# tenpy/cyten

Measured on AMD Instinct MI355X. Metric: block-sparse tdot+SVD GFLOP/s (fp64), higher is better.
Workload: dtype f64

## Files before the change

cyten_amd/csrc/blocked_qr.h:

```cpp
#pragma once
#include "common.h"

namespace cyb {

constexpr int NBK = 32;

struct BqrMat {
    double* Ac;
    int64_t ld;
    int32_t m, n, k;
    double* V;
    double* T;
    double* tau;
    double* scratch;
    int64_t scr_half;
    int64_t scr_total = 0;
    int32_t v_zeroed = 0;
    double* ctl = nullptr;
    double* parts = nullptr;
    double stop_rel2 = 0.0;
    int32_t reflect_always = 0;
};

size_t bqr_aux_bytes(int64_t m, int64_t n, int64_t ld, int64_t kc);
size_t bqr_carve(BqrMat& q, char* base, int64_t kc);

int bqr_strip_slots(int64_t rows);

int bqr_factor(cyb_ctx_t ctx, const std::vector<BqrMat>& mats);

struct BqrTarget {
    int32_t mat;
    double* C;
    int64_t ldc;
    int32_t kc;
    int32_t n_pan = -1;
};
int bqr_apply_q(cyb_ctx_t ctx, const std::vector<BqrMat>& mats, const std::vector<BqrTarget>& targets);
int bqr_apply_q_pair(cyb_ctx_t ctx, const std::vector<BqrMat>& mats, const std::vector<BqrTarget>& targets, size_t n_first);

struct XposeDesc {
    const double* in;
    double* out;
    int64_t ldi, ldo;
    int32_t R, C, upper, rlim;
    int32_t plain, pad;
    const int32_t* idx = nullptr;
};
int xpose_batched(cyb_ctx_t ctx, const std::vector<XposeDesc>& descs);
struct EyeDesc {
    double* C;
    int64_t ld;
    int32_t m, kc;
    int32_t col0, pad;
};
int eye_cols_batched(cyb_ctx_t ctx, const std::vector<EyeDesc>& descs);

}
```

cyten_amd/csrc/blocked_qr.hip:

```cpp
#include "blocked_qr.h"

#include <algorithm>
#include <cstdlib>
#include <utility>

namespace cyb {
namespace {

#define GLOBAL_AS __attribute__((address_space(1)))
typedef GLOBAL_AS double* gp;
typedef const GLOBAL_AS double* gcp;
typedef double d4 __attribute__((ext_vector_type(4)));

constexpr int PNT = 512;
constexpr int PNW = PNT / 64;

__device__ __forceinline__ double wave_sum(double v)
{
#pragma unroll
    for (int o = 32; o > 0; o >>= 1) v += __shfl_xor(v, o);
    return v;
}

struct PanelDesc {
    double* Ac;
    double* V;
    double* T;
    double* tau;
    int64_t ld;
    int32_t m, j0, pw, pad;
    double* ctl = nullptr;
    const double* parts = nullptr;
    double rel2 = 0.0;
    int32_t n_parts = 0, step = 0;
};
constexpr int PANEL_V_ZEROED = 1;
constexpr int PANEL_REFLECT_ALWAYS = 2;

__global__ void __launch_bounds__(PNT) qr_panel_kernel(const PanelDesc* __restrict__ descs)
{
    __shared__ double red[PNW];
    __shared__ double s_tau, s_scale;
    __shared__ double Ts[NBK][NBK + 1];
    __shared__ double z[NBK];
    __shared__ double taus[NBK];
    const PanelDesc d = descs[blockIdx.x];
    const int tid = threadIdx.x, lane = tid & 63, wave = tid >> 6;
    gp Ac = (gp)d.Ac;
    gp V = (gp)d.V;
    const int64_t ld = d.ld;
    const int m = d.m, j0 = d.j0, pw = d.pw;
    for (int e = tid; e < NBK * (NBK + 1); e += PNT) (&Ts[0][0])[e] = 0.0;

    for (int jj = 0; jj < pw; ++jj) {
        const int col = j0 + jj;
        gp x = Ac + (int64_t)col * ld + col;
        const int L = m - col;
        double mx = 0.0;
        for (int i = 1 + tid; i < L; i += PNT) mx = fmax(mx, fabs(x[i]));
#pragma unroll
        for (int o = 32; o > 0; o >>= 1) mx = fmax(mx, __shfl_xor(mx, o));
        if (lane == 0) red[wave] = mx;
        __syncthreads();
        mx = 0.0;
#pragma unroll
        for (int q = 0; q < PNW; ++q) mx = fmax(mx, red[q]);
        __syncthreads();
        double ss = 0.0;
        if (mx > 1e-290) {
            const double inv = 1.0 / mx;
            for (int i = 1 + tid; i < L; i += PNT) {
                const double t = x[i] * inv;
                ss += t * t;
            }
        }
        ss = wave_sum(ss);
        if (lane == 0) red[wave] = ss;
        __syncthreads();
        if (tid == 0) {
            double tot = 0.0;
            for (int q = 0; q < PNW; ++q) tot += red[q];
            const double xnorm = mx * sqrt(tot);
            const double alpha = x[0];
            double t = 0.0, scale = 0.0, beta = alpha;
            if (xnorm != 0.0) {
                beta = -copysign(hypot(alpha, xnorm), alpha);
// ... 291 lines not shown
        gcp src = (gcp)Ac + (int64_t)j0 * ld + (ok ? row : j0);
#pragma unroll
        for (int c = 0; c < NBK; ++c) P[q][c] = src[(int64_t)(c < pw ? c : pw - 1) * ld];
#pragma unroll
        for (int c = 0; c < NBK; ++c) {
            asm volatile("" : "+v"(P[q][c]));
            P[q][c] = (ok && c < pw) ? P[q][c] : 0.0;
        }
    }
    for (int e = tid; e < NBK * (NBK + 1); e += NT) (&sh.Zs[0][0])[e] = 0.0;
    __syncthreads();

    panel_steps<RPT, NT>(P, sh, d, tid, std::make_integer_sequence<int, NBK>{});
#pragma unroll
    for (int q = 0; q < RPT; ++q) {
        const int row = j0 + tid + NT * q;
        if (row < m) {
            gp pa = Ac + (int64_t)j0 * ld + row;
            gp pv = V + (int64_t)j0 * ld + row;
#pragma unroll
            for (int c = 0; c < NBK; ++c)
                if (c < pw) {
                    pa[(int64_t)c * ld] = P[q][c];
                    pv[(int64_t)c * ld] = (q > 0 || tid > c) ? P[q][c] : (tid == c ? 1.0 : 0.0);
                }
        }
    }
    for (int64_t e = tid; e < ((d.pad & PANEL_V_ZEROED) ? 0 : (int64_t)j0 * pw); e += NT) {
        const int c = (int)(e / j0), row = (int)(e % j0);
        V[(int64_t)(j0 + c) * ld + row] = 0.0;
    }
    __syncthreads();
    if (tid < NBK) {
        double trow[NBK];
#pragma unroll
        for (int j = 0; j < NBK; ++j) {
            double acc = 0.0;
#pragma unroll
            for (int l = 0; l < j; ++l) acc += trow[l] * sh.Zs[l][j];
            const double tj = j < pw ? sh.taus[j] : 0.0;
            trow[j] = (tid < j) ? -tj * acc : (tid == j ? tj : 0.0);
            sh.Ts[tid][j] = trow[j];
        }
    }
    __syncthreads();

    for (int e = tid; e < NBK * NBK; e += NT) ((gp)d.T)[e] = sh.Ts[e / NBK][e % NBK];
}

template <int NT, typename Desc>
__device__ __forceinline__ bool panel_stop_check(const Desc& d, double* red, int tid, bool writer = true)
{
    if (!d.ctl) return false;
    gp ctl = (gp)d.ctl;
    const double stopped = ctl[0];
    if (stopped != 0.0) return (double)d.step >= stopped - 1.0;
    if (d.n_parts <= 0) return false;
    gcp parts = (gcp)d.parts;
    double t = 0.0;
    for (int i = tid; i < d.n_parts; i += NT) t += parts[i];
#pragma unroll
    for (int o = 32; o > 0; o >>= 1) t += __shfl_xor(t, o);
    if ((tid & 63) == 0) red[tid >> 6] = t;
    __syncthreads();
    double sum = 0.0;
#pragma unroll
    for (int w = 0; w < NT / 64; ++w) sum += red[w];
    const double ref = fmax(ctl[1], sum);
    const bool stop = sum <= d.rel2 * ref;
    __syncthreads();
    if (tid == 0 && writer) {
        if (stop) ctl[0] = (double)d.step + 1.0;
        else ctl[1] = ref;
    }
    return stop;
}

__global__ void __launch_bounds__(RP_NT) qr_panel_reg_kernel(const PanelDesc* __restrict__ descs)
{
    __shared__ PanelShared sh;
    const PanelDesc d = descs[blockIdx.x];
    if (panel_stop_check<RP_NT>(d, &sh.wsum[0][0], (int)threadIdx.x)) return;
    panel_reg_body<RP_RPT>(d, sh, (int)threadIdx.x);
}
struct PanelDescM {
    double* Ac;
    double* V;
    double* T;
    double* tau;
    double* xchg;
    unsigned int* ticket;
    unsigned int* err;
    int64_t ld;
    int32_t m, j0, pw, vzero;
    int32_t wg, n_wg, pad0, pad1;
    double* ctl = nullptr;
    const double* parts = nullptr;
    double rel2 = 0.0;
    int32_t n_parts = 0, step = 0;
};
constexpr int RPM_ROWS = RP_NT * RP_RPT;

template <int JJ>
__device__ __forceinline__ void panel_step_multi(double (&P)[RP_RPT][NBK], PanelShared& sh, const PanelDescM& d, int tid)
{
    if (JJ >= d.pw) return;
    const int lane = tid & 63, wave = tid >> 6;
    const int j0 = d.j0, rbase = d.j0 + d.wg * RPM_ROWS;
    const int prow = j0 + JJ;
    constexpr int pb = JJ & 1;
#pragma unroll
    for (int h = 0; h < 2; ++h) {
        double part[16];
#pragma unroll
        for (int c = 0; c < 16; ++c) part[c] = 0.0;
#pragma unroll
        for (int q = 0; q < RP_RPT; ++q) {
            const int row = rbase + tid + RP_NT * q;
            const double x = (row <= prow) ? 0.0 : P[q][JJ];
#pragma unroll
            for (int c = 0; c < 16; ++c) part[c] += x * P[q][h * 16 + c];
        }
        const double r = reduce_scatter16(part, lane);
        if ((lane & 3) == 0) {
            const int idx = ((lane >> 5) & 1) * 8 + ((lane >> 4) & 1) * 4 + ((lane >> 3) & 1) * 2 + ((lane >> 2) & 1);
            sh.wred[pb][wave][h * 16 + idx] = r;
        }
    }
#pragma unroll
    for (int q = 0; q < RP_RPT; ++q)
        if (rbase + tid + RP_NT * q == prow) {
#pragma unroll
            for (int c = 0; c < NBK; ++c) sh.rowb[pb][c] = P[q][c];
        }
    __syncthreads();
    if (tid < NBK) {
        double t = 0.0;
#pragma unroll
        for (int w = 0; w < RP_NW; ++w) t += sh.wred[pb][w][tid];
        double* slot = d.xchg + ((size_t)JJ * d.n_wg + d.wg) * 64;
        __hip_atomic_store(slot + tid, t, __ATOMIC_RELAXED, __HIP_MEMORY_SCOPE_AGENT);
        if (d.wg == 0) __hip_atomic_store(slot + 32 + tid, sh.rowb[pb][tid], __ATOMIC_RELAXED, __HIP_MEMORY_SCOPE_AGENT);
        asm volatile("s_waitcnt vmcnt(0)" ::: "memory");
        if (tid == 0) {
            __hip_atomic_fetch_add(d.ticket + JJ, 1u, __ATOMIC_RELAXED, __HIP_MEMORY_SCOPE_AGENT);
            const unsigned long long t0 = wall_clock64();
            while (__hip_atomic_load(d.ticket + JJ, __ATOMIC_RELAXED, __HIP_MEMORY_SCOPE_AGENT) < (unsigned int)d.n_wg) {
                if (wall_clock64() - t0 > 100000000ull || __hip_atomic_load(d.err, __ATOMIC_RELAXED, __HIP_MEMORY_SCOPE_AGENT)) {
                    __hip_atomic_store(d.err, 1u, __ATOMIC_RELAXED, __HIP_MEMORY_SCOPE_AGENT);
                    break;
                }
            }
        }
        asm volatile("" ::: "memory");
        __builtin_amdgcn_wave_barrier();
        double tot = 0.0;
        for (int w = 0; w < d.n_wg; ++w)
            tot += __hip_atomic_load(d.xchg + ((size_t)JJ * d.n_wg + w) * 64 + tid, __ATOMIC_RELAXED, __HIP_MEMORY_SCOPE_AGENT);
        sh.wsum[pb][tid] = tot;
        sh.rowb[pb][tid] = __hip_atomic_load(d.xchg + (size_t)JJ * d.n_wg * 64 + 32 + tid, __ATOMIC_RELAXED, __HIP_MEMORY_SCOPE_AGENT);
    }
    __syncthreads();
    const double alpha = sh.rowb[pb][JJ];
    const double xn2 = fma(alpha * alpha, (d.vzero & PANEL_REFLECT_ALWAYS) ? 1e-40 : 0.0, sh.wsum[pb][JJ]);
    double tau = 0.0, scale = 0.0, beta = alpha;
    if (xn2 > 1e-290) {
// ... 687 lines not shown
#pragma unroll
        for (int q = 0; q < 4; ++q) {
            const int c = c0 + ty + 8 * q, r = r0 + tx;
            tile[ty + 8 * q][tx] = (c < d.C && r < d.R) ? in[(int64_t)(d.idx ? cidx[ty + 8 * q] : c) * d.ldi + r] : 0.0;
        }
        __syncthreads();
#pragma unroll
        for (int q = 0; q < 4; ++q) {
            const int r = r0 + ty + 8 * q, c = c0 + tx;
            if (r < d.R && c < d.C) {
                double v = tile[tx][ty + 8 * q];
                if (d.upper && (r > c || r >= d.rlim)) v = 0.0;
                out[(int64_t)r * d.ldo + c] = v;
            }
        }
    }
}

__global__ void __launch_bounds__(256) eye_cols_kernel(const EyeDesc* __restrict__ descs)
{
    const EyeDesc d = descs[blockIdx.y];
    gp C = (gp)d.C;
    const int64_t tot = (int64_t)d.m * d.kc;
    for (int64_t e = (int64_t)blockIdx.x * 256 + threadIdx.x; e < tot; e += (int64_t)gridDim.x * 256) {
        const int64_t c = e / d.m, i = e % d.m;
        C[c * d.ld + i] = (i == c + d.col0) ? 1.0 : 0.0;
    }
}

}

int xpose_batched(cyb_ctx_t ctx, const std::vector<XposeDesc>& descs)
{
    if (descs.empty()) return CYB_OK;
    void* d = nullptr;
    CYB_TRY(ctx->upload(descs.data(), sizeof(XposeDesc) * descs.size(), &d));
    hipLaunchKernelGGL(xpose_kernel, dim3(helper_grid_x(descs.size()), (unsigned)descs.size()), dim3(256), 0, ctx->stream, static_cast<const XposeDesc*>(d));
    CYB_HIP(hipGetLastError());
    return CYB_OK;
}

int eye_cols_batched(cyb_ctx_t ctx, const std::vector<EyeDesc>& descs)
{
    if (descs.empty()) return CYB_OK;
    void* d = nullptr;
    CYB_TRY(ctx->upload(descs.data(), sizeof(EyeDesc) * descs.size(), &d));
    hipLaunchKernelGGL(eye_cols_kernel, dim3(64, (unsigned)descs.size()), dim3(256), 0, ctx->stream, static_cast<const EyeDesc*>(d));
    CYB_HIP(hipGetLastError());
    return CYB_OK;
}

constexpr int kWSplit = 8;
static inline int w_split(int64_t mr)
{
    static const int env = getenv("CYB_QR_WSPLIT") ? atoi(getenv("CYB_QR_WSPLIT")) : 0;
    if (env > 0) return (int)std::min<int64_t>(std::min(env, kWSplit), std::max<int64_t>(1, (mr + 255) / 256));
    return mr >= 2600 ? 4 : mr >= 1800 ? 3 : mr >= 700 ? 2 : 1;
}

static inline bool use_strips()
{
    static const bool off = getenv("CYB_QR_GEMM_UPDATE") != nullptr;
    return !off;
}
static void add_strips(std::vector<StripDesc>& out, double* C, int64_t ldc, int64_t ncols, const double* V, int64_t ldv,
                       const double* T, int64_t mr, int pw, int transT, int64_t next_tag = -1)
{
    for (int64_t c0 = 0; c0 < ncols; c0 += NBK)
        out.push_back(StripDesc{C + (size_t)c0 * ldc, V, T, ldc, ldv, (int32_t)mr, (int32_t)std::min<int64_t>(NBK, ncols - c0), pw, transT,
                                c0 == 0 && next_tag >= 0 ? next_tag + 1 : 0});
}
static void sort_strips(std::vector<StripDesc>& v)
{
    std::stable_sort(v.begin(), v.end(), [](const StripDesc& a, const StripDesc& b) { return a.mr > b.mr; });
}

constexpr int kChunkRowsMin = 192;
static const int kChunkRowsChoices[] = {192, 256, 384, 512, 768, 1024, 1536};
static int strip_split_mode()
{
    static const int v = getenv("CYB_QR_CHUNK_ROWS") ? atoi(getenv("CYB_QR_CHUNK_ROWS")) : -1;
    return v < 0 ? -1 : v / 16 * 16;
}
int bqr_strip_slots(int64_t rows)
{
    if (strip_split_mode() == 0) return 1;
    const int ch = strip_split_mode() > 0 ? std::min(strip_split_mode(), kChunkRowsMin) : kChunkRowsMin;
    return (int)std::max<int64_t>(1, (rows + ch - 1) / ch);
}
static int strip_chunk_share(int mr, int ch)
{
    if (ch <= 0 || mr <= ch) return std::max(mr, 1);
    const int ns = (mr + ch - 1) / ch;
    return ((mr + ns - 1) / ns + 15) / 16 * 16;
}
static int strip_chunks(int mr, int ch)
{
    const int share = strip_chunk_share(mr, ch);
    return std::max(1, (mr + share - 1) / share);
}
static int choose_chunk_rows(const std::vector<std::pair<int, int>>& strips, int n_cu)
{
    const int mode = strip_split_mode();
    if (mode == 0) return 0;
    if (mode > 0) return mode;
    int64_t n_strips = 0;
    for (const auto& s : strips) n_strips += s.second;
    if (n_strips == 0 || n_strips * 4 > (int64_t)n_cu * 3) return 0;
    static const int ch_min = getenv("CYB_QR_CHUNK_MIN") ? atoi(getenv("CYB_QR_CHUNK_MIN")) : kChunkRowsMin;
    for (int ch : kChunkRowsChoices) {
        if (ch < ch_min) continue;
        int64_t tot = 0;
        bool any = false;
        for (const auto& s : strips) {
            const int c = strip_chunks(s.first, ch);
            tot += (int64_t)c * s.second;
            any = any || c > 1;
        }
        if (tot <= n_cu) return any ? ch : 0;
    }
    return 0;
}
static void make_chunks(const std::vector<StripDesc>& sd, double* wbase, int ch, std::vector<ChunkDesc>& out)
{
    out.clear();
    size_t slot_base = 0;
    for (const StripDesc& d : sd) {
        const int share = strip_chunk_share(d.mr, ch), nch = strip_chunks(d.mr, ch);
        for (int sl = 0; sl < nch; ++sl) {
            const int r0 = sl * share;
            out.push_back(ChunkDesc{d.C + r0, d.V + r0, d.T, wbase + slot_base * (size_t)(NBK * NBK), d.ldc, d.ldv, std::min(share, d.mr - r0), d.nc, d.pw,
                                    d.transT, sl, nch, r0, d.step, d.ctl, d.part_out ? d.part_out + sl : nullptr});
        }
        slot_base += (size_t)nch;
    }
}

static int wide_mode()
{
    static const int v = getenv("CYB_QR_APPLY_WIDE") ? (atoi(getenv("CYB_QR_APPLY_WIDE")) != 0 ? 1 : 0) : -1;
    return v;
}
static int wide_width()
{
    static const int v = [] {
        const int e = getenv("CYB_QR_APPLY_WIDTH") ? atoi(getenv("CYB_QR_APPLY_WIDTH")) : 128;
        return (e == 64 || e == 256) ? e : 128;
    }();
    return v;
}
constexpr int64_t kWideMinK = 256, kWideMinKc = 256, kWideMinCols = 4096;
static bool wide_target(const BqrMat& q, const BqrTarget& t)
{
    const int mode = wide_mode();
    if (mode == 0 || q.k <= NBK || t.kc <= 0) return false;
    if (q.ctl && q.stop_rel2 > 0.0 && t.n_pan < 0) return false;
    if (mode == 1) return true;
    return q.k >= kWideMinK && t.kc >= kWideMinKc;
}
static size_t scratch_doubles(int64_t m, int64_t n, int64_t kc)
{
    const size_t strips = (size_t)(1 + kWSplit) * NBK * (size_t)std::max<int64_t>(std::max(n, kc), 1);
    const size_t wide = (size_t)w_split(m) * (size_t)wide_width() * (size_t)std::max<int64_t>(kc, 1);
    return std::max(strips, wide);
}

// ... 33 lines not shown
    const bool strips = use_strips();
    const bool lookahead = !strips && want_la && max_pan >= 6 && ctx->aux(&side) == CYB_OK;
    struct Step {
        size_t off_pd = 0, off_pdr = 0;
        unsigned n_pd = 0, n_pdr = 0;
        GemmStaged s1, s3;
        GemmStaged r1, r3;
        bool has_rest = false;
        size_t off_sd = 0;
        unsigned n_sd = 0;
        bool fused = false;
        bool norm = false;
        unsigned n_la = 0;
        size_t off_pn = 0;
        size_t off_cd = 0;
        unsigned n_cd = 0;
        int wave = 0;
        size_t off_pdm = 0;
        unsigned n_pdm = 0;
    };
    std::vector<Step> steps;
    std::vector<char> image;
    auto put = [&image](const void* src, size_t bytes) {
        const size_t off = (image.size() + 255) / 256 * 256;
        image.resize(off + bytes);
        memcpy(image.data() + off, src, bytes);
        return off;
    };
    static const bool no_fuse = getenv("CYB_QR_FUSE") == nullptr;
    static const int fuse_rows = getenv("CYB_QR_FUSE_ROWS") ? atoi(getenv("CYB_QR_FUSE_ROWS")) : 768;
    std::vector<char> fused(mats.size(), 0);
    static const bool la_on = getenv("CYB_QR_LA") && atoi(getenv("CYB_QR_LA")) != 0;
    static const int la_min_rows = getenv("CYB_QR_LA_MIN") ? atoi(getenv("CYB_QR_LA_MIN")) : 4 * RP_WAVE_ROWS;
    unsigned int* la_flags = nullptr;
    const int la_err = (int)mats.size();
    bool la_used = false;
    static const bool no_multi = getenv("CYB_QR_NOMULTI") != nullptr;
    std::vector<size_t> x_off(mats.size(), 0);
    size_t x_bytes = 0, n_multi_wg = 0;
    const size_t t_bytes = (sizeof(unsigned int) * NBK * mats.size() + 255) / 256 * 256;
    for (size_t qi = 0; qi < mats.size(); ++qi) {
        const int wmax = (mats[qi].m + RPM_ROWS - 1) / RPM_ROWS;
        if (mats[qi].m > RPM_ROWS && std::min(mats[qi].m, mats[qi].n) > 0) {
            x_off[qi] = t_bytes + 256 + x_bytes;
            x_bytes += sizeof(double) * NBK * (size_t)wmax * 64;
            n_multi_wg += (size_t)wmax;
        }
    }
    const bool multi = !no_multi && x_bytes > 0 && n_multi_wg <= (size_t)ctx->n_cu;
    char* xbase = nullptr;
    bool la_any = false;
    if (la_on && use_strips())
        for (const auto& q : mats) la_any = la_any || (q.k > NBK && q.m - NBK > la_min_rows);
    if (multi || la_any) {
        const size_t x_total = multi ? (t_bytes + 256 + x_bytes + 255) / 256 * 256 : 0;
        void* xw = nullptr;
        CYB_TRY(ctx->workspace(x_total + 256 + sizeof(unsigned int) * (mats.size() + 1), &xw, 3));
        xbase = static_cast<char*>(xw);
        if (multi) CYB_HIP(hipMemsetAsync(xbase + t_bytes, 0, 256, ctx->stream));
        if (la_any) {
            la_flags = reinterpret_cast<unsigned int*>(xbase + x_total);
            CYB_HIP(hipMemsetAsync(la_flags, 0, sizeof(unsigned int) * (mats.size() + 1), ctx->stream));
        }
    }
    const bool multi_ok = multi;
    static const bool no_stop = getenv("CYB_QR_NOSTOP") != nullptr;
    static const bool no_reg_g = getenv("CYB_QR_PANEL_GLOBAL") != nullptr;
    auto stoppable = [&](const BqrMat& q) {
        return !no_stop && strips && !no_reg_g && q.ctl && q.parts && q.stop_rel2 > 0.0 && (q.m <= RP_NT * RP_RPT || multi_ok);
    };
    const bool split = strips && strip_split_mode() != 0 && no_fuse && !la_on;
    double* wsplit = nullptr;
    if (split) {
        size_t n_ch = 0;
        for (const auto& q : mats) n_ch += (size_t)((q.n + NBK - 1) / NBK) * (size_t)bqr_strip_slots(q.m);
        void* w = nullptr;
        CYB_TRY(ctx->workspace(sizeof(double) * NBK * NBK * std::max<size_t>(n_ch, 1), &w, 4));
        wsplit = static_cast<double*>(w);
    }
    std::vector<int> n_parts_prev(mats.size(), 0);
    static const int stop_every = std::max(1, getenv("CYB_QR_STOP_EVERY") ? atoi(getenv("CYB_QR_STOP_EVERY")) : 2);
    bool all_done = false;
    int last_rest = -1;
    const int side_cu = ctx->n_cu - (ctx->n_cu + 15) / 16;
    int chunk = lookahead ? max_pan : 2;
    for (int c0 = 0; c0 < max_pan && !all_done; c0 += chunk, chunk *= 3) {
    const int c1 = std::min(max_pan, c0 + chunk);
    steps.clear();
    image.clear();
    for (int p = c0; p < c1; ++p) {
        std::vector<PanelDesc> pd, pd_reg, pd_next;
        std::vector<PanelDescM> pdm;
        std::vector<StripDesc> sd;
        GemmBatch g1, g3, h1, h3;
        int n_active = 0;
        int max_m = 0;
        for (const auto& q : mats)
            if (p * NBK < q.k) max_m = std::max(max_m, q.m);
        const bool step_fuse = !no_fuse && max_m <= fuse_rows;
        const bool step_la = la_on && strips && !step_fuse && la_flags != nullptr;
        bool step_has_la = false;
        bool step_norm = false;
        int step_ch = 0;
        if (split && !step_fuse) {
            std::vector<std::pair<int, int>> cnt;
            for (const auto& q : mats) {
                const int j0 = p * NBK;
                if (j0 >= q.k) continue;
                const int64_t nt = q.n - (j0 + std::min(NBK, q.k - j0));
                if (nt > 0) cnt.push_back({q.m - j0, (int)((nt + NBK - 1) / NBK)});
            }
            step_ch = choose_chunk_rows(cnt, ctx->n_cu);
        }
        for (size_t qi = 0; qi < mats.size(); ++qi) {
            const auto& q = mats[qi];
            const int j0 = p * NBK;
            if (j0 >= q.k) continue;
            ++n_active;
            const int pw = std::min(NBK, q.k - j0);
            static const bool no_reg = getenv("CYB_QR_PANEL_GLOBAL") != nullptr;
            if (fused[qi]) fused[qi] = 0;
            else if (!no_reg && q.m - j0 <= RP_NT * RP_RPT) {
                pd_reg.push_back(PanelDesc{q.Ac, q.V, q.T + (size_t)p * NBK * NBK, q.tau, q.ld, q.m, j0, pw, pflags(q)});
                if (stoppable(q)) {
                    PanelDesc& d = pd_reg.back();
                    d.ctl = q.ctl;
                    d.parts = q.parts;
                    d.rel2 = q.stop_rel2;
                    d.n_parts = n_parts_prev[qi];
                    d.step = p;
                }
            } else if (multi && !no_reg) {
                const int n_wg = (q.m - j0 + RPM_ROWS - 1) / RPM_ROWS;
                for (int w = 0; w < n_wg; ++w)
                {
                    pdm.push_back(PanelDescM{q.Ac, q.V, q.T + (size_t)p * NBK * NBK, q.tau, reinterpret_cast<double*>(xbase + x_off[qi]),
                                             reinterpret_cast<unsigned int*>(xbase) + qi * NBK, reinterpret_cast<unsigned int*>(xbase + t_bytes),
                                             q.ld, q.m, j0, pw, pflags(q), w, n_wg, 0, 0});
                    if (stoppable(q)) {
                        PanelDescM& d = pdm.back();
                        d.ctl = q.ctl;
                        d.parts = q.parts;
                        d.rel2 = q.stop_rel2;
                        d.n_parts = n_parts_prev[qi];
                        d.step = p;
                    }
                }
            } else
                pd.push_back(PanelDesc{q.Ac, q.V, q.T + (size_t)p * NBK * NBK, q.tau, q.ld, q.m, j0, pw, pflags(q) & PANEL_REFLECT_ALWAYS});
            const int j1 = j0 + pw;
            const int64_t nt = q.n - j1, mr = q.m - j0;
            const int parts_lag = n_parts_prev[qi];
            n_parts_prev[qi] = 0;
            if (nt <= 0) continue;
            double* W1 = q.scratch + q.scr_half;
            const double* Vp = q.V + (size_t)j0 * q.ld + j0;
            const double* Tp = q.T + (size_t)p * NBK * NBK;
            if (strips) {
                int64_t tag = -1;
                if (step_fuse && !no_reg && !stoppable(q) && j1 < q.k && q.m - j1 <= RP_NT * RP_RPT_FUSED) {
                    tag = (int64_t)pd_next.size();
                    pd_next.push_back(PanelDesc{q.Ac, q.V, q.T + (size_t)(p + 1) * NBK * NBK, q.tau, q.ld, q.m, j1, std::min(NBK, q.k - j1), pflags(q)});
                    fused[qi] = 1;
                } else if (step_la && !no_reg && j1 < q.k && q.m - j1 <= RP_NT * RP_RPT && q.m - j1 > la_min_rows) {
                    tag = (int64_t)pd_next.size();
                    pd_next.push_back(PanelDesc{q.Ac, q.V, q.T + (size_t)(p + 1) * NBK * NBK, q.tau, q.ld, q.m, j1, std::min(NBK, q.k - j1), pflags(q)});
                    if (stoppable(q)) {
                        const bool measure = p % stop_every == stop_every - 1;
                        PanelDesc& d = pd_next.back();
                        d.ctl = q.ctl;
                        d.parts = q.parts;
                        d.rel2 = q.stop_rel2;
                        d.n_parts = measure ? 0 : parts_lag;
                        d.step = p + 1;
                    }
                    fused[qi] = 1;
                    step_has_la = true;
                }
                const size_t s_begin = sd.size();
                add_strips(sd, q.Ac + (size_t)j1 * q.ld + j0, q.ld, nt, Vp, q.ld, Tp, mr, pw, 1, tag);
                if (stoppable(q)) {
                    const bool measure = p % stop_every == stop_every - 1;
                    const int nch = strip_chunks((int)mr, step_ch);
                    for (size_t si = s_begin; si < sd.size(); ++si) {
                        sd[si].ctl = q.ctl;
                        sd[si].part_out = measure ? q.parts + (si - s_begin) * (size_t)nch : nullptr;
                        sd[si].step = p;
                    }
                    if (measure) {
                        n_parts_prev[qi] = (int)(sd.size() - s_begin) * nch;
                        step_norm = true;
                    }
                }
                continue;
            }
            const int ns = w_split(mr);
            const int64_t chunk = ((mr + ns - 1) / ns + 15) / 16 * 16;
            const int64_t nn = lookahead ? std::min<int64_t>(NBK, nt) : nt;
            auto add = [&](GemmBatch& a1, GemmBatch& a3, int64_t c0, int64_t nc, size_t scr_off) {
                if (nc <= 0) return;
                double* At = q.Ac + (size_t)(j1 + c0) * q.ld + j0;
                const int32_t seg0 = (int32_t)a3.segs.size();
                for (int sidx = 0; sidx < ns; ++sidx) {
                    const int64_t r0 = chunk * sidx, rows = std::min(chunk, mr - r0);
                    if (rows <= 0) break;
                    double* W2s = W1 + (size_t)sidx * q.scr_half + scr_off;
                    a1.add_post(W2s, pw, nc, nc, Vp + r0, q.ld, 1, At + r0, 1, q.ld, rows, 1.0, 0.0, Tp, 1, NBK);
                    a3.segs.push_back(cyb_gemm_seg{W2s, Vp, pw, 1, nc, q.ld, 1});
                }
                a3.probs.push_back(cyb_gemm_prob{At, nc, mr, q.ld, seg0, (int32_t)a3.segs.size(), -1.0, 1.0});
            };
            add(g1, g3, 0, nn, 0);
            add(h1, h3, nn, nt - nn, (size_t)NBK * NBK);
        }
        if (n_active == 0) {
            all_done = true;
            break;
        }
        Step st;
        st.n_pd = (unsigned)pd.size();
        st.n_pdr = (unsigned)pd_reg.size();
        if (st.n_pd) st.off_pd = put(pd.data(), sizeof(PanelDesc) * pd.size());
        if (st.n_pdr) st.off_pdr = put(pd_reg.data(), sizeof(PanelDesc) * pd_reg.size());
        st.n_pdm = (unsigned)pdm.size();
        if (st.n_pdm) st.off_pdm = put(pdm.data(), sizeof(PanelDescM) * pdm.size());
        static const bool no_wave = getenv("CYB_QR_NOWAVE") != nullptr;
        int max_rows = 0;
        for (const auto& d : pd_reg) max_rows = std::max(max_rows, d.m - d.j0);
        st.wave = (no_wave || st.n_pdr == 0) ? 0 : max_rows <= RP_WAVE_ROWS ? 1 : max_rows <= 2 * RP_WAVE_ROWS ? 2 : max_rows <= 4 * RP_WAVE_ROWS ? 4 : 0;
        if (!sd.empty()) {
            sort_strips(sd);
            st.n_sd = (unsigned)sd.size();
            st.fused = !pd_next.empty() && !step_has_la;
            st.norm = step_norm;
            const size_t off_pn = pd_next.empty() ? 0 : put(pd_next.data(), sizeof(PanelDesc) * pd_next.size());
            const size_t off_sd = (image.size() + 255) / 256 * 256;
            if (step_has_la) {
                st.n_la = (unsigned)pd_next.size();
                st.off_pn = off_pn;
                la_used = true;
            } else
                for (auto& d : sd)
                    if (d.next_off) d.next_off = (int64_t)(off_pn + (size_t)(d.next_off - 1) * sizeof(PanelDesc)) - (int64_t)off_sd;
            st.off_sd = put(sd.data(), sizeof(StripDesc) * sd.size());
            if (step_ch > 0 && !st.fused && !st.n_la) {
                std::vector<ChunkDesc> cd;
                make_chunks(sd, wsplit, step_ch, cd);
                st.n_cd = (unsigned)cd.size();
                st.off_cd = put(cd.data(), sizeof(ChunkDesc) * cd.size());
            }
        }
        if (!g1.empty()) {
            CYB_TRY(g1.stage(ctx, image, st.s1));
            CYB_TRY(g3.stage(ctx, image, st.s3));
        }
        if (!h1.empty()) {
            CYB_TRY(h1.stage(ctx, image, st.r1));
            CYB_TRY(h3.stage(ctx, image, st.r3));
            st.has_rest = true;
        }
        steps.push_back(st);
    }
    if (steps.empty()) break;
    void* d_image = nullptr;
    CYB_TRY(ctx->upload(image.data(), image.size(), &d_image));
    char* dbase = static_cast<char*>(d_image);
    if (lookahead) CYB_TRY(ctx->events(2 * steps.size()));
    for (size_t p = 0; p < steps.size(); ++p) {
        const Step& st = steps[p];
        if (st.n_pd)
            hipLaunchKernelGGL(qr_panel_kernel, dim3(st.n_pd), dim3(PNT), 0, ctx->stream,
                               reinterpret_cast<const PanelDesc*>(dbase + st.off_pd));
        if (st.n_pdm) {
            CYB_HIP(hipMemsetAsync(xbase, 0, t_bytes, ctx->stream));
            hipLaunchKernelGGL(qr_panel_multi_kernel, dim3(st.n_pdm), dim3(RP_NT), 0, ctx->stream,
                               reinterpret_cast<const PanelDescM*>(dbase + st.off_pdm));
        }
        if (st.n_pdr && st.wave == 1)
            hipLaunchKernelGGL(qr_panel_wave_kernel, dim3(st.n_pdr), dim3(64), 0, ctx->stream,
                               reinterpret_cast<const PanelDesc*>(dbase + st.off_pdr));
        else if (st.n_pdr && st.wave == 2)
            hipLaunchKernelGGL(qr_panel_wave2_kernel, dim3(st.n_pdr), dim3(128), 0, ctx->stream,
                               reinterpret_cast<const PanelDesc*>(dbase + st.off_pdr));
        else if (st.n_pdr && st.wave == 4)
            hipLaunchKernelGGL(qr_panel_wave4_kernel, dim3(st.n_pdr), dim3(256), 0, ctx->stream,
                               reinterpret_cast<const PanelDesc*>(dbase + st.off_pdr));
        else if (st.n_pdr)
            hipLaunchKernelGGL(qr_panel_reg_kernel, dim3(st.n_pdr), dim3(RP_NT), 0, ctx->stream,
                               reinterpret_cast<const PanelDesc*>(dbase + st.off_pdr));
        CYB_HIP(hipGetLastError());
        if (lookahead && st.has_rest) {
            hipEvent_t evP = ctx->ev_pool[2 * p], evR = ctx->ev_pool[2 * p + 1];
            CYB_HIP(hipEventRecord(evP, ctx->stream));
            CYB_HIP(hipStreamWaitEvent(side, evP, 0));
            CYB_TRY(gemm_launch_staged(ctx, st.r1, d_image, side, side_cu));
            CYB_TRY(gemm_launch_staged(ctx, st.r3, d_image, side, side_cu));
            CYB_HIP(hipEventRecord(evR, side));
            if (last_rest >= 0) CYB_HIP(hipStreamWaitEvent(ctx->stream, ctx->ev_pool[2 * (size_t)last_rest + 1], 0));
            last_rest = (int)p;
        } else if (lookahead && last_rest >= 0) {
            CYB_HIP(hipStreamWaitEvent(ctx->stream, ctx->ev_pool[2 * (size_t)last_rest + 1], 0));
            last_rest = -1;
        }
        if (st.n_sd) {
            const StripDesc* sdp = reinterpret_cast<const StripDesc*>(dbase + st.off_sd);
            const PanelDesc* pnp = reinterpret_cast<const PanelDesc*>(dbase + st.off_pn);
            const unsigned la_tag = (unsigned)(c0 + (int)p + 1);
            const PanelDesc* no_pn = nullptr;
            unsigned int* no_fl = nullptr;
            if (st.n_cd) {
                const ChunkDesc* cdp = reinterpret_cast<const ChunkDesc*>(dbase + st.off_cd);
                hipLaunchKernelGGL(strip_w1_kernel, dim3(st.n_cd), dim3(ST_NT), 0, ctx->stream, cdp);
                if (st.norm) hipLaunchKernelGGL(strip_apply_kernel<true>, dim3(st.n_cd), dim3(ST_NT), 0, ctx->stream, cdp);
                else hipLaunchKernelGGL(strip_apply_kernel<false>, dim3(st.n_cd), dim3(ST_NT), 0, ctx->stream, cdp);
            } else if (st.n_la && st.norm)
                hipLaunchKernelGGL((reflector_strip_kernel<false, true, true>), dim3(st.n_sd + st.n_la), dim3(ST_NT), 0, ctx->stream, sdp,
                                   (int)st.n_sd, pnp, la_flags, la_tag, la_err);
            else if (st.n_la)
                hipLaunchKernelGGL((reflector_strip_kernel<false, false, true>), dim3(st.n_sd + st.n_la), dim3(ST_NT), 0, ctx->stream, sdp,
                                   (int)st.n_sd, pnp, la_flags, la_tag, la_err);
            else if (st.fused)
                hipLaunchKernelGGL(reflector_strip_kernel<true>, dim3(st.n_sd), dim3(ST_NT), 0, ctx->stream, sdp, (int)st.n_sd, no_pn, no_fl, 0u, 0);
            else if (st.norm)
                hipLaunchKernelGGL((reflector_strip_kernel<false, true>), dim3(st.n_sd), dim3(ST_NT), 0, ctx->stream, sdp, (int)st.n_sd, no_pn, no_fl, 0u, 0);
            else
                hipLaunchKernelGGL(reflector_strip_kernel<false>, dim3(st.n_sd), dim3(ST_NT), 0, ctx->stream, sdp, (int)st.n_sd, no_pn, no_fl, 0u, 0);
            CYB_HIP(hipGetLastError());
        }
        CYB_TRY(gemm_launch_staged(ctx, st.s1, d_image));
        CYB_TRY(gemm_launch_staged(ctx, st.s3, d_image));
    }
    }
    if (last_rest >= 0) CYB_HIP(hipStreamWaitEvent(ctx->stream, ctx->ev_pool[2 * (size_t)last_rest + 1], 0));
    if (la_used) {
        unsigned int h_err = 0;
        CYB_HIP(hipMemcpyAsync(&h_err, la_flags + la_err, sizeof(unsigned int), hipMemcpyDeviceToHost, ctx->stream));
        CYB_HIP(hipStreamSynchronize(ctx->stream));
        if (h_err) {
            set_error("blocked QR: a look-ahead panel workgroup waited more than a second for its strip");
            return CYB_ERR_HIP;
        }
    }
    if (multi) {
        unsigned int h_err = 0;
        CYB_HIP(hipMemcpyAsync(&h_err, xbase + t_bytes, sizeof(unsigned int), hipMemcpyDeviceToHost, ctx->stream));
        CYB_HIP(hipStreamSynchronize(ctx->stream));
        if (h_err) {
            set_error("blocked QR: a workgroup of the multi-workgroup panel kernel waited more than a second for its partners");
            return CYB_ERR_HIP;
        }
    }
    return CYB_OK;
}

static int apply_q_strips(cyb_ctx_t ctx, const std::vector<BqrMat>& mats, const std::vector<BqrTarget>& targets)
{
    int max_pan = 0;
    for (const auto& t : targets) max_pan = std::max(max_pan, (mats[(size_t)t.mat].k + NBK - 1) / NBK);
    const bool strips = use_strips();
    struct Step {
        GemmStaged s1, s3;
        size_t off_sd = 0;
        unsigned n_sd = 0;
        size_t off_cd = 0;
        unsigned n_cd = 0;
    };
    const bool split = strips && strip_split_mode() != 0;
    double* wsplit = nullptr;
    if (split) {
        size_t n_ch = 0;
        for (const auto& t : targets) n_ch += (size_t)((t.kc + NBK - 1) / NBK) * (size_t)bqr_strip_slots(mats[(size_t)t.mat].m);
        void* w = nullptr;
        CYB_TRY(ctx->workspace(sizeof(double) * NBK * NBK * std::max<size_t>(n_ch, 1), &w, 4));
        wsplit = static_cast<double*>(w);
    }
    std::vector<Step> steps;
    std::vector<char> image;
    int chunk = 2;
    for (int c0 = max_pan - 1; c0 >= 0; c0 -= chunk, chunk *= 3) {
    const int c1 = std::max(-1, c0 - chunk);
    steps.clear();
    image.clear();
    for (int p = c0; p > c1; --p) {
        GemmBatch g1, g3;
        std::vector<StripDesc> sd;
        for (const auto& t : targets) {
            const BqrMat& q = mats[(size_t)t.mat];
            const int j0 = p * NBK;
            if (j0 >= q.k || t.kc <= 0) continue;
            const int pw = std::min(NBK, q.k - j0);
            const int64_t mr = q.m - j0;
            double* W1 = q.scratch + q.scr_half;
            CYB_REQUIRE((int64_t)NBK * t.kc <= q.scr_half, "bqr_apply_q: target wider than the carved scratch");
            const double* Vp = q.V + (size_t)j0 * q.ld + j0;
            double* Ct = t.C + j0;
            const double* Tp = q.T + (size_t)p * NBK * NBK;
            if (strips) {
                const size_t s_begin = sd.size();
                add_strips(sd, Ct, t.ldc, t.kc, Vp, q.ld, Tp, mr, pw, 0);
                if (q.ctl && q.stop_rel2 > 0.0)
                    for (size_t si = s_begin; si < sd.size(); ++si) {
                        sd[si].ctl = q.ctl;
                        sd[si].step = p;
                    }
                continue;
            }
            const int ns = w_split(mr);
            const int64_t chunk = ((mr + ns - 1) / ns + 15) / 16 * 16;
            const int32_t seg0 = (int32_t)g3.segs.size();
            for (int sidx = 0; sidx < ns; ++sidx) {
                const int64_t r0 = chunk * sidx, rows = std::min(chunk, mr - r0);
                if (rows <= 0) break;
                double* W2s = W1 + (size_t)sidx * q.scr_half;
                g1.add_post(W2s, pw, t.kc, t.kc, Vp + r0, q.ld, 1, Ct + r0, 1, t.ldc, rows, 1.0, 0.0, Tp, NBK, 1);
                g3.segs.push_back(cyb_gemm_seg{W2s, Vp, pw, 1, t.kc, q.ld, 1});
// ... 252 lines not shown
```

cyten_amd/csrc/qr_householder.hip:

```cpp
#include "blocked_qr.h"

#include <algorithm>
#include <cstdlib>

namespace {

#define GLOBAL_AS __attribute__((address_space(1)))
typedef GLOBAL_AS double* gp;
typedef const GLOBAL_AS double* gcp;

constexpr int QNT = 512;
constexpr int QNW = QNT / 64;

struct QrWork {
    const double* A;
    int64_t lda;
    int32_t m, n, k, kq;
    double* Ac;
    double* Qc;
    double* tau;
    double* Q;
    int64_t ldq;
    double* R;
    int64_t ldr;
// ... 110 lines not shown
    for (int64_t e = tid; e < (int64_t)m * kq; e += QNT) {
        const int i = (int)(e / kq), c = (int)(e % kq);
        ((gp)w.Q)[(int64_t)i * w.ldq + c] = Qc[(int64_t)c * m + i];
    }
}

}

static constexpr int64_t kBlockedMin = 96;

static int qr_blocked(cyb_ctx_t ctx, const std::vector<cyb_qr_desc>& ds)
{
    using namespace cyb;
    if (ds.empty()) return CYB_OK;
    auto al = [](size_t b) { return (b + 255) / 256 * 256; };
    std::vector<BqrMat> mats(ds.size());
    std::vector<size_t> oA(ds.size()), oAux(ds.size()), oC(ds.size());
    std::vector<int> kq(ds.size());
    size_t off = 0;
    for (size_t i = 0; i < ds.size(); ++i) {
        const auto& d = ds[i];
        const int64_t k = std::min(d.m, d.n);
        kq[i] = (int)(d.full ? d.m : k);
        oA[i] = off;
        off += al(sizeof(double) * (size_t)d.m * d.n);
        oAux[i] = off;
        off += bqr_aux_bytes(d.m, d.n, d.m, kq[i]);
        oC[i] = off;
        off += al(sizeof(double) * (size_t)d.m * kq[i]);
    }
    void* ws = nullptr;
    CYB_TRY(ctx->workspace(off, &ws, 1));
    char* base = static_cast<char*>(ws);
    std::vector<XposeDesc> x_in, x_r, x_q;
    std::vector<EyeDesc> eyes;
    std::vector<BqrTarget> targets;
    for (size_t i = 0; i < ds.size(); ++i) {
        const auto& d = ds[i];
        BqrMat& q = mats[i];
        q.Ac = reinterpret_cast<double*>(base + oA[i]);
        q.ld = d.m;
        q.m = (int)d.m;
        q.n = (int)d.n;
        q.k = (int)std::min(d.m, d.n);
        bqr_carve(q, base + oAux[i], kq[i]);
        double* Cq = reinterpret_cast<double*>(base + oC[i]);
        x_in.push_back(XposeDesc{d.A, q.Ac, d.lda, d.m, (int)d.n, (int)d.m, 0, 0, 0, 0});
        x_r.push_back(XposeDesc{q.Ac, d.R, d.m, d.ldr, d.full ? (int)d.m : q.k, (int)d.n, 1, q.k, 0, 0});
        eyes.push_back(EyeDesc{Cq, d.m, (int)d.m, kq[i], 0, 0});
        targets.push_back(BqrTarget{(int)i, Cq, d.m, kq[i]});
        x_q.push_back(XposeDesc{Cq, d.Q, d.m, d.ldq, (int)d.m, kq[i], 0, 0, 0, 0});
    }
    CYB_TRY(xpose_batched(ctx, x_in));
    CYB_TRY(bqr_factor(ctx, mats));
    CYB_TRY(xpose_batched(ctx, x_r));
    CYB_TRY(eye_cols_batched(ctx, eyes));
    CYB_TRY(bqr_apply_q(ctx, mats, targets));
    CYB_TRY(xpose_batched(ctx, x_q));
    return CYB_OK;
}

static int qr_batched_impl(cyb_ctx_t ctx, const cyb_qr_desc* descs, int64_t nmat)
{
    CYB_REQUIRE(ctx, "cyb_qr_batched_f64: ctx is NULL");
    CYB_REQUIRE(nmat >= 0 && (nmat == 0 || descs), "cyb_qr_batched_f64: bad descriptor list");
    std::vector<QrWork> works;
    std::vector<size_t> oAc, oQc, oTau;
    size_t off = 0;
    auto take = [&](size_t bytes) {
        const size_t o = off;
        off += (bytes + 255) / 256 * 256;
        return o;
    };
    std::vector<cyb_qr_desc> big;
    for (int64_t b = 0; b < nmat; ++b) {
        const cyb_qr_desc& d = descs[b];
        CYB_REQUIRE(d.m >= 0 && d.n >= 0 && d.m < (1 << 30) && d.n < (1 << 30), "qr block %lld: bad shape", (long long)b);
        if (d.m == 0 || d.n == 0) continue;
        CYB_REQUIRE(d.A && d.Q && d.R, "qr block %lld: NULL pointer", (long long)b);
        {
            const int64_t kq_ = d.full ? d.m : std::min(d.m, d.n);
            CYB_REQUIRE(d.lda >= d.n && d.ldq >= kq_ && d.ldr >= d.n, "qr block %lld: leading dimension too small", (long long)b);
        }
        if (std::min(d.m, d.n) >= kBlockedMin && getenv("CYB_QR_UNBLOCKED") == nullptr) {
            big.push_back(d);
            continue;
        }
        QrWork w;
        w.A = d.A;
        w.lda = d.lda;
        w.m = (int)d.m;
        w.n = (int)d.n;
        w.k = (int)std::min(d.m, d.n);
        w.kq = d.full ? (int)d.m : w.k;
        w.r_rows = d.full ? (int)d.m : w.k;
        CYB_REQUIRE(d.lda >= d.n && d.ldq >= w.kq && d.ldr >= d.n, "qr block %lld: leading dimension too small", (long long)b);
        w.Q = d.Q;
        w.ldq = d.ldq;
        w.R = d.R;
        w.ldr = d.ldr;
        w.pad = 0;
        w.Ac = w.Qc = w.tau = nullptr;
        oAc.push_back(take(sizeof(double) * (size_t)d.m * d.n));
        oQc.push_back(take(sizeof(double) * (size_t)d.m * w.kq));
        oTau.push_back(take(sizeof(double) * (size_t)w.k));
        works.push_back(w);
    }
    CYB_TRY(qr_blocked(ctx, big));
    if (works.empty()) return CYB_OK;
    void* ws = nullptr;
    CYB_TRY(ctx->workspace(off, &ws));
    char* base = static_cast<char*>(ws);
    for (size_t i = 0; i < works.size(); ++i) {
        works[i].Ac = reinterpret_cast<double*>(base + oAc[i]);
        works[i].Qc = reinterpret_cast<double*>(base + oQc[i]);
        works[i].tau = reinterpret_cast<double*>(base + oTau[i]);
    }
    void* d_w = nullptr;
    CYB_TRY(ctx->upload(works.data(), sizeof(QrWork) * works.size(), &d_w));
    hipLaunchKernelGGL(qr_householder_kernel, dim3((unsigned)works.size()), dim3(QNT), 0, ctx->stream,
                       static_cast<const QrWork*>(d_w));
    CYB_HIP(hipGetLastError());
    return CYB_OK;
}

extern "C" int cyb_qr_batched_f64(cyb_ctx_t ctx, const cyb_qr_desc* descs, int64_t nmat)
{
    CYB_REQUIRE(ctx, "cyb_qr_batched_f64: ctx is NULL");
    CYB_REQUIRE(nmat >= 0 && (nmat == 0 || descs), "cyb_qr_batched_f64: bad descriptor list");
    std::vector<cyb::MatRef> refs;
    std::vector<int64_t> which;
    for (int64_t b = 0; b < nmat; ++b)
        if (descs[b].m > 0 && descs[b].n > 0 && descs[b].A) {
            refs.push_back(cyb::MatRef{descs[b].A, descs[b].lda, descs[b].m, descs[b].n});
            which.push_back(b);
        }
    std::vector<double> amax;
    CYB_TRY(cyb::matrix_amax(ctx, refs, amax));
    std::vector<cyb_qr_desc> mod;
    std::vector<void*> temps;
    std::vector<cyb::ScaleJob> pre, post;
    for (size_t k = 0; k < refs.size(); ++k) {
        const double sc = cyb::range_scale(amax[k]);
        if (sc == 1.0) continue;
        if (mod.empty()) mod.assign(descs, descs + nmat);
        cyb_qr_desc& d = mod[(size_t)which[k]];
        void* t = nullptr;
        CYB_HIP(hipMalloc(&t, sizeof(double) * (size_t)d.m * (size_t)d.n));
        temps.push_back(t);
        pre.push_back(cyb::ScaleJob{d.A, d.lda, static_cast<double*>(t), d.n, d.m, d.n, sc});
        d.A = static_cast<const double*>(t);
        d.lda = d.n;
        const int64_t r_rows = d.full ? d.m : std::min(d.m, d.n);
        post.push_back(cyb::ScaleJob{d.R, d.ldr, d.R, d.ldr, r_rows, d.n, 1.0 / sc});
    }
    if (mod.empty()) return qr_batched_impl(ctx, descs, nmat);
    int st = cyb::scale_copy_batched(ctx, pre);
    if (st == CYB_OK) st = qr_batched_impl(ctx, mod.data(), nmat);
    if (st == CYB_OK) st = cyb::scale_copy_batched(ctx, post);
    (void)hipStreamSynchronize(ctx->stream);
    for (void* t : temps) (void)hipFree(t);
    return st;
}
```

Measured before the change: 5559.

## Add split-column panel QR kernel pipelining two column halves across workgroup halves

Adds a new 512-thread panel factorization kernel where each half of the workgroup holds 16 of the 32 panel columns in registers. The two halves pipeline reflector generation and application across 34 phases, with the lead half computing the next reflector while the other half applies earlier ones. The kernel is routed in for panels whose row count exceeds the wave kernels' limit but fits the register panel kernel, replacing qr_panel_reg_kernel there. It also adds a route tracing option and an env override for the blocked-QR threshold. The pipelined phase scheme adds sync points per phase and heavy register use.

New measurement: 5491. -1.2%, worse.

```diff
diff --git a/cyten_amd/csrc/blocked_qr.h b/cyten_amd/csrc/blocked_qr.h
--- a/cyten_amd/csrc/blocked_qr.h
+++ b/cyten_amd/csrc/blocked_qr.h
@@ -26,6 +26,7 @@
 size_t bqr_carve(BqrMat& q, char* base, int64_t kc);
 
 int bqr_strip_slots(int64_t rows);
+int bqr_panel_route(int max_rows, bool no_wave, bool no_split);
 
 int bqr_factor(cyb_ctx_t ctx, const std::vector<BqrMat>& mats);
 
diff --git a/cyten_amd/csrc/blocked_qr.hip b/cyten_amd/csrc/blocked_qr.hip
--- a/cyten_amd/csrc/blocked_qr.hip
+++ b/cyten_amd/csrc/blocked_qr.hip
@@ -2,6 +2,7 @@
 
 #include <algorithm>
 #include <cstdlib>
+#include <string>
 #include <utility>
 
 namespace cyb {
@@ -459,6 +460,217 @@
     const PanelDesc d = descs[blockIdx.x];
     if (panel_stop_check<RP_NT>(d, &sh.wsum[0][0], (int)threadIdx.x)) return;
     panel_reg_body<RP_RPT>(d, sh, (int)threadIdx.x);
+}
+constexpr int SP_NT = 512;
+constexpr int SP_HT = SP_NT / 2;
+constexpr int SP_RPT = 6;
+constexpr int SP_HC = NBK / 2;
+constexpr int SP_ROWS = SP_HT * SP_RPT;
+static_assert(SP_HC == 16 && SP_ROWS == RP_NT * RP_RPT, "the split panel kernel serves the rows of qr_panel_reg_kernel");
+
+struct SplitShared {
+    double xb[3][SP_RPT * SP_HT];
+    double wred[2][2][SP_HT / 64][SP_HC];
+    double rowb[2][NBK];
+    double scales[NBK];
+    double taus[NBK];
+    double Zs[NBK][NBK + 1];
+    double Ts[NBK][NBK + 1];
+};
+
+template <int S>
+struct SplitPhase {
+    static constexpr int LC = S < 16 ? S : (S == 16 || S == 33) ? -1 : S - 1;
+    static constexpr int LH = S < 16 ? 0 : 1;
+    static constexpr int FR = S == 0 ? -1 : S <= 16 ? S - 1 : S == 17 ? -1 : S - 2;
+    static constexpr int FH = S <= 16 ? 1 : 0;
+};
+
+template <int S>
+__device__ __forceinline__ void split_phase(double (&P)[SP_RPT][SP_HC], SplitShared& sh, const PanelDesc& d, int tid)
+{
+    using Ph = SplitPhase<S>;
+    constexpr int LC = Ph::LC, FR = Ph::FR;
+    constexpr int ph = S & 1;
+    const int pw = d.pw;
+    const bool lead_on = LC >= 0 && LC < pw;
+    const bool follow_on = FR >= 0 && FR < pw && (Ph::FH == 0 || pw > SP_HC);
+    if (!lead_on && !follow_on) return;
+    const int half = tid >> 8, th = tid & (SP_HT - 1), lane = tid & 63, simd = th >> 6;
+    const bool lead = lead_on && half == Ph::LH;
+    const bool follow = follow_on && half == Ph::FH;
+    constexpr int C = LC >= 0 ? LC : 0, HL = C & (SP_HC - 1);
+    constexpr int F = FR >= 0 ? FR : 0;
+    if (lead || follow) {
+        const int piv = lead ? C : F;
+        double x[SP_RPT];
+        if (lead) {
+#pragma unroll
+            for (int q = 0; q < SP_RPT; ++q) {
+                x[q] = (q == 0 && th <= C) ? 0.0 : P[q][HL];
+                sh.xb[C % 3][q * SP_HT + th] = x[q];
+            }
+        } else {
+#pragma unroll
+            for (int q = 0; q < SP_RPT; ++q) x[q] = sh.xb[F % 3][q * SP_HT + th];
+        }
+        double part[SP_HC];
+#pragma unroll
+        for (int c = 0; c < SP_HC; ++c) part[c] = 0.0;
+#pragma unroll
+        for (int q = 0; q < SP_RPT; ++q)
+#pragma unroll
+            for (int c = 0; c < SP_HC; ++c) part[c] += x[q] * P[q][c];
+        const double r = reduce_scatter16(part, lane);
+        if ((lane & 3) == 0) {
+            const int idx = ((lane >> 5) & 1) * 8 + ((lane >> 4) & 1) * 4 + ((lane >> 3) & 1) * 2 + ((lane >> 2) & 1);
+            sh.wred[ph][half][simd][idx] = r;
+        }
+        if (th == piv) {
+#pragma unroll
+            for (int c = 0; c < SP_HC; ++c) sh.rowb[ph][half * SP_HC + c] = P[0][c];
+        }
+    }
+    __syncthreads();
+    if (!(lead || follow)) return;
+    const int lc = lane & (SP_HC - 1);
+    double ws = 0.0;
+#pragma unroll
+    for (int w = 0; w < SP_HT / 64; ++w) ws += sh.wred[ph][half][w][lc];
+    const double rb = sh.rowb[ph][half * SP_HC + lc];
+    if (lead) {
+        const int prow = d.j0 + C;
+        const double alpha = __hiloint2double(__builtin_amdgcn_readlane(__double2hiint(rb), HL), __builtin_amdgcn_readlane(__double2loint(rb), HL));
+        const double xn2_raw = __hiloint2double(__builtin_amdgcn_readlane(__double2hiint(ws), HL), __builtin_amdgcn_readlane(__double2loint(ws), HL));
+        const double xn2 = fma(alpha * alpha, (d.pad & PANEL_REFLECT_ALWAYS) ? 1e-40 : 0.0, xn2_raw);
+        double tau = 0.0, scale = 0.0, beta = alpha;
+        if (xn2 > 1e-290) {
+            beta = -copysign(sqrt(alpha * alpha + xn2), alpha);
+            tau = (beta - alpha) / beta;
+            scale = 1.0 / (alpha - beta);
+        }
+        double v[SP_RPT];
+#pragma unroll
+        for (int q = 0; q < SP_RPT; ++q) {
+            const double xq = P[q][HL];
+            if (q == 0) {
+                const bool below = th > C;
+                const bool pivot = th == C;
+                v[q] = below ? xq * scale : (pivot ? 1.0 : 0.0);
+                P[q][HL] = below ? v[q] : (pivot ? beta : xq);
+            } else {
+                v[q] = xq * scale;
+                P[q][HL] = v[q];
+            }
+        }
+        const double z = rb + scale * ws;
+        const double tl = tau * z;
+        const int tlo = __double2loint(tl), thi = __double2hiint(tl);
+#pragma unroll
+        for (int c = HL + 1; c < SP_HC; ++c) {
+            const double t = __hiloint2double(__builtin_amdgcn_readlane(thi, c), __builtin_amdgcn_readlane(tlo, c));
+#pragma unroll
+            for (int q = 0; q < SP_RPT; ++q) P[q][c] -= t * v[q];
+        }
+        if (th < HL) sh.Zs[Ph::LH * SP_HC + th][C] = z;
+        if (th == 0) {
+            sh.taus[C] = tau;
+            sh.scales[C] = scale;
+            ((gp)d.tau)[prow] = tau;
+        }
+    } else {
+        const double tau = sh.taus[F], scale = sh.scales[F];
+        const double z = rb + scale * ws;
+        if (Ph::FH == 0) {
+            if (th < SP_HC) sh.Zs[th][F] = z;
+        } else {
+            double v[SP_RPT];
+#pragma unroll
+            for (int q = 0; q < SP_RPT; ++q) v[q] = sh.xb[F % 3][q * SP_HT + th] * scale;
+            if (th == F) v[0] = 1.0;
+            const double tl = tau * z;
+            const int tlo = __double2loint(tl), thi = __double2hiint(tl);
+#pragma unroll
+            for (int c = 0; c < SP_HC; ++c) {
+                const double t = __hiloint2double(__builtin_amdgcn_readlane(thi, c), __builtin_amdgcn_readlane(tlo, c));
+#pragma unroll
+                for (int q = 0; q < SP_RPT; ++q) P[q][c] -= t * v[q];
+            }
+        }
+    }
+}
+
+template <int... Ss>
+__device__ __forceinline__ void split_phases(double (&P)[SP_RPT][SP_HC], SplitShared& sh, const PanelDesc& d, int tid,
+                                             std::integer_sequence<int, Ss...>)
+{
+    (split_phase<Ss>(P, sh, d, tid), ...);
+}
+
+__global__ void __launch_bounds__(SP_NT) qr_panel_split_kernel(const PanelDesc* __restrict__ descs)
+{
+    __shared__ SplitShared sh;
+    const PanelDesc d = descs[blockIdx.x];
+    const int tid = (int)threadIdx.x;
+    if (panel_stop_check<SP_NT>(d, &sh.xb[0][0], tid)) return;
+    gp Ac = (gp)d.Ac;
+    gp V = (gp)d.V;
+    const int64_t ld = d.ld;
+    const int m = d.m, j0 = d.j0, pw = d.pw;
+    const int half = tid >> 8, th = tid & (SP_HT - 1), c0 = half * SP_HC;
+    double P[SP_RPT][SP_HC];
+#pragma unroll
+    for (int q = 0; q < SP_RPT; ++q) {
+        const int row = j0 + th + SP_HT * q;
+        const bool ok = row < m;
+        gcp src = (gcp)Ac + (int64_t)j0 * ld + (ok ? row : j0);
+#pragma unroll
+        for (int c = 0; c < SP_HC; ++c) P[q][c] = src[(int64_t)(c0 + c < pw ? c0 + c : pw - 1) * ld];
+#pragma unroll
+        for (int c = 0; c < SP_HC; ++c) {
+            asm volatile("" : "+v"(P[q][c]));
+            P[q][c] = (ok && c0 + c < pw) ? P[q][c] : 0.0;
+        }
+    }
+    for (int e = tid; e < NBK * (NBK + 1); e += SP_NT) (&sh.Zs[0][0])[e] = 0.0;
+    __syncthreads();
+
+    split_phases(P, sh, d, tid, std::make_integer_sequence<int, 34>{});
+    int thw = th;
+    asm volatile("" : "+v"(thw));
+#pragma unroll
+    for (int q = 0; q < SP_RPT; ++q) {
+        const int row = j0 + thw + SP_HT * q;
+        if (row < m) {
+            gp pa = Ac + (int64_t)j0 * ld + row;
+            gp pv = V + (int64_t)j0 * ld + row;
+#pragma unroll
+            for (int c = 0; c < SP_HC; ++c)
+                if (c0 + c < pw) {
+                    pa[(int64_t)(c0 + c) * ld] = P[q][c];
+                    pv[(int64_t)(c0 + c) * ld] = (q > 0 || th > c0 + c) ? P[q][c] : (th == c0 + c ? 1.0 : 0.0);
+                }
+        }
+    }
+    for (int64_t e = tid; e < ((d.pad & PANEL_V_ZEROED) ? 0 : (int64_t)j0 * pw); e += SP_NT) {
+        const int c = (int)(e / j0), row = (int)(e % j0);
+        V[(int64_t)(j0 + c) * ld + row] = 0.0;
+    }
+    __syncthreads();
+    if (tid < NBK) {
+        double trow[NBK];
+#pragma unroll
+        for (int j = 0; j < NBK; ++j) {
+            double acc = 0.0;
+#pragma unroll
+            for (int l = 0; l < j; ++l) acc += trow[l] * sh.Zs[l][j];
+            const double tj = j < pw ? sh.taus[j] : 0.0;
+            trow[j] = (tid < j) ? -tj * acc : (tid == j ? tj : 0.0);
+            sh.Ts[tid][j] = trow[j];
+        }
+    }
+    __syncthreads();
+    for (int e = tid; e < NBK * NBK; e += SP_NT) ((gp)d.T)[e] = sh.Ts[e / NBK][e % NBK];
 }
 struct PanelDescM {
     double* Ac;
@@ -1312,6 +1524,16 @@
     static const int v = getenv("CYB_QR_CHUNK_ROWS") ? atoi(getenv("CYB_QR_CHUNK_ROWS")) : -1;
     return v < 0 ? -1 : v / 16 * 16;
 }
+int bqr_panel_route(int max_rows, bool no_wave, bool no_split)
+{
+    if (no_wave) return 0;
+    if (max_rows <= RP_WAVE_ROWS) return 1;
+    if (max_rows <= 2 * RP_WAVE_ROWS) return 2;
+    if (max_rows <= 4 * RP_WAVE_ROWS) return 4;
+    return (!no_split && max_rows <= SP_ROWS) ? 8 : 0;
+}
+extern "C" int cybqr_panel_route(int max_rows, int no_wave, int no_split) { return bqr_panel_route(max_rows, no_wave != 0, no_split != 0); }
+
 int bqr_strip_slots(int64_t rows)
 {
     if (strip_split_mode() == 0) return 1;
@@ -1511,6 +1733,8 @@
     static const int stop_every = std::max(1, getenv("CYB_QR_STOP_EVERY") ? atoi(getenv("CYB_QR_STOP_EVERY")) : 2);
     bool all_done = false;
     int last_rest = -1;
+    static const bool trace = getenv("CYB_QR_TRACE_ROUTE") != nullptr;
+    std::string trace_line;
     const int side_cu = ctx->n_cu - (ctx->n_cu + 15) / 16;
     int chunk = lookahead ? max_pan : 2;
     for (int c0 = 0; c0 < max_pan && !all_done; c0 += chunk, chunk *= 3) {
@@ -1656,7 +1880,8 @@
         static const bool no_wave = getenv("CYB_QR_NOWAVE") != nullptr;
         int max_rows = 0;
         for (const auto& d : pd_reg) max_rows = std::max(max_rows, d.m - d.j0);
-        st.wave = (no_wave || st.n_pdr == 0) ? 0 : max_rows <= RP_WAVE_ROWS ? 1 : max_rows <= 2 * RP_WAVE_ROWS ? 2 : max_rows <= 4 * RP_WAVE_ROWS ? 4 : 0;
+        static const bool no_split = getenv("CYB_QR_NOSPLIT") != nullptr;
+        st.wave = st.n_pdr == 0 ? 0 : bqr_panel_route(max_rows, no_wave, no_split);
         if (!sd.empty()) {
             sort_strips(sd);
             st.n_sd = (unsigned)sd.size();
@@ -1714,10 +1939,16 @@
         else if (st.n_pdr && st.wave == 4)
             hipLaunchKernelGGL(qr_panel_wave4_kernel, dim3(st.n_pdr), dim3(256), 0, ctx->stream,
                                reinterpret_cast<const PanelDesc*>(dbase + st.off_pdr));
+        else if (st.n_pdr && st.wave == 8)
+            hipLaunchKernelGGL(qr_panel_split_kernel, dim3(st.n_pdr), dim3(SP_NT), 0, ctx->stream,
+                               reinterpret_cast<const PanelDesc*>(dbase + st.off_pdr));
         else if (st.n_pdr)
             hipLaunchKernelGGL(qr_panel_reg_kernel, dim3(st.n_pdr), dim3(RP_NT), 0, ctx->stream,
                                reinterpret_cast<const PanelDesc*>(dbase + st.off_pdr));
         CYB_HIP(hipGetLastError());
+        if (trace)
+            trace_line += std::string(" ") + (st.n_pd ? "g" : "") + (st.n_pdm ? "m" : "") + (st.n_pdr ? std::to_string(st.wave) : std::string()) +
+                          (st.n_pd + st.n_pdm + st.n_pdr ? "" : "-");
         if (lookahead && st.has_rest) {
             hipEvent_t evP = ctx->ev_pool[2 * p], evR = ctx->ev_pool[2 * p + 1];
             CYB_HIP(hipEventRecord(evP, ctx->stream));
@@ -1760,6 +1991,7 @@
         CYB_TRY(gemm_launch_staged(ctx, st.s3, d_image));
     }
     }
+    if (trace) fprintf(stderr, "[cyb] bqr_factor: %zu matrices, panel kernels per step:%s\n", mats.size(), trace_line.c_str());
     if (last_rest >= 0) CYB_HIP(hipStreamWaitEvent(ctx->stream, ctx->ev_pool[2 * (size_t)last_rest + 1], 0));
     if (la_used) {
         unsigned int h_err = 0;
diff --git a/cyten_amd/csrc/qr_householder.hip b/cyten_amd/csrc/qr_householder.hip
--- a/cyten_amd/csrc/qr_householder.hip
+++ b/cyten_amd/csrc/qr_householder.hip
@@ -216,7 +216,8 @@
             const int64_t kq_ = d.full ? d.m : std::min(d.m, d.n);
             CYB_REQUIRE(d.lda >= d.n && d.ldq >= kq_ && d.ldr >= d.n, "qr block %lld: leading dimension too small", (long long)b);
         }
-        if (std::min(d.m, d.n) >= kBlockedMin && getenv("CYB_QR_UNBLOCKED") == nullptr) {
+        static const int64_t blocked_min = getenv("CYB_QR_BLOCKED_MIN") ? std::max(1, atoi(getenv("CYB_QR_BLOCKED_MIN"))) : kBlockedMin;
+        if (std::min(d.m, d.n) >= blocked_min && getenv("CYB_QR_UNBLOCKED") == nullptr) {
             big.push_back(d);
             continue;
         }
```
